# hahnyuan/PTQ4ViT

Measured on AMD Instinct MI355X. Metric: calibration throughput (wrapped modules calibrated per second), ViT-B/224 W8A8, 32 calibration images, higher is better.
Workload: dtype int8

## Files before the change

include/ptq4vit_hip_debug.h:

```cpp
#ifndef PTQ4VIT_HIP_DEBUG_H
#define PTQ4VIT_HIP_DEBUG_H

#include <stdint.h>

#ifdef __cplusplus
extern "C" {
#endif

int p4v_debug_set_variant(int variant, int force_generic);
int p4v_debug_set_tuning(int key, int value);
int p4v_debug_topk_rows(const float* d_mass, int segs, int n, int k, int32_t* d_idx, void* stream);

#ifdef __cplusplus
}
#endif
#endif
```

ptq4vit_amd/_lib.py:

```python
import ctypes as C
import os

_HERE = os.path.dirname(os.path.abspath(__file__))
LIB_PATH = os.environ.get("P4V_LIB") or os.path.join(_HERE, "csrc", "libptq4vit_hip.so")

METRICS = {
    "L1_norm": 0,
    "L2_norm": 1,
    "linear_weighted_L2_norm": 2,
    "square_weighted_L2_norm": 3,
    "hessian": 4,
    "cosine": 5,
}


class LinearDesc(C.Structure):
    _fields_ = [(n, C.c_int32) for n in (
        "batch", "tokens", "in_features", "out_features", "n_V", "n_H", "n_a", "w_bit", "a_bit", "metric",
        "eq_n", "search_round", "twin_postgelu", "init_layerwise", "has_bias", "reserved")]


class MatMulDesc(C.Structure):
    _fields_ = ([(n, C.c_int32) for n in ("batch", "heads", "M", "K", "N")] + [("_pad0", C.c_int32)] +
                [("a_stride", C.c_int64 * 4), ("b_stride", C.c_int64 * 4)] +
# ... 16 lines not shown
                ("memo_hits", C.c_int64), ("memo_misses", C.c_int64),
                ("sweep7_ms", C.c_double), ("sweep7_launches", C.c_int64), ("sweep7_macs", C.c_double), ("sweep7_alg_macs", C.c_double),
                ("sweep7_twin_ms", C.c_double), ("sweep7_twin_launches", C.c_int64), ("event_overhead_ms", C.c_double)]


class LaunchRecord(C.Structure):
    _fields_ = [("kind", C.c_int32), ("stage", C.c_int32), ("grid_x", C.c_int32), ("grid_z", C.c_int32),
                ("ms", C.c_double), ("ops", C.c_double), ("alg_ops", C.c_double), ("alg_bytes", C.c_double)]


LAUNCH_KINDS = {0: "k_sweep<int8>", 1: "k_sweep<float>", 2: "k_sweep6", 3: "k_sweep7", 4: "k_sweep7 (twin)", 5: "k_sweep4/5", 6: "k_sweep9",
                7: "k_sweep8", 8: "k_sweep2g", 9: "k_sweep2", 11: "k_sos_split", 12: "k_bound", 13: "k_slice_b", 14: "k_slice_a"}
LAUNCH_STAGES = {0: "full", 1: "A", 2: "B1", 3: "B2", 4: "A2"}


class PlaneDesc(C.Structure):
    _fields_ = [("rows", C.c_int64), ("cols", C.c_int64), ("cols_padded", C.c_int64), ("rows_per_scale", C.c_int64),
                ("mode", C.c_int32), ("lo", C.c_int32), ("hi", C.c_int32), ("qmax", C.c_int32),
                ("const_scale", C.c_float), ("reserved", C.c_int32)]


class ExportDesc(C.Structure):
    _fields_ = [("dims", C.c_int32 * 4), ("src_stride", C.c_int64 * 4),
                ("scale1_stride", C.c_int64 * 4), ("scale1_div", C.c_int32 * 4),
                ("scale2_stride", C.c_int64 * 4), ("scale2_div", C.c_int32 * 4),
                ("scale2_const", C.c_float),
                ("mode", C.c_int32), ("lo1", C.c_int32), ("hi1", C.c_int32), ("lo2", C.c_int32), ("hi2", C.c_int32),
                ("qmax", C.c_int32), ("reserved", C.c_int32)]


class GroupJob(C.Structure):
    _fields_ = [("kind", C.c_int32), ("status", C.c_int32), ("desc", C.c_void_p), ("inp", C.c_void_p * 5), ("mult", C.c_void_p),
                ("out", C.c_void_p * 3), ("workspace", C.c_void_p), ("workspace_bytes", C.c_size_t)]


JOB_LINEAR, JOB_MATMUL, JOB_CONV = 0, 1, 2
PLANE_SYM, PLANE_SOS_HI, PLANE_SOS_LO, PLANE_TWIN = 1, 2, 3, 4
EXPORT_SYM_I8, EXPORT_SYM_F32, EXPORT_GELU_U8, EXPORT_SOS_U8 = 0, 1, 2, 3


EXPORTS = [
    "p4v_version", "p4v_last_error",
    "p4v_linear_workspace_bytes", "p4v_linear_calibrate",
    "p4v_matmul_workspace_bytes", "p4v_matmul_calibrate",
    "p4v_conv_workspace_bytes", "p4v_conv_calibrate",
    "p4v_calibrate_group", "p4v_launch_counters",
    "p4v_linear_quant_forward", "p4v_matmul_quant_forward",
    "p4v_amax_init_linear", "p4v_linear_search_w", "p4v_linear_search_a",
    "p4v_amax_init_matmul", "p4v_matmul_search_A", "p4v_sos_search_split", "p4v_matmul_search_B",
    "p4v_amax_init_conv", "p4v_conv_search_w_channelwise", "p4v_conv_search_w_layerwise", "p4v_conv_search_a",
    "p4v_score_argmax_gather",
    "p4v_quantize_i8", "p4v_pack_plane_i8", "p4v_fake_quant", "p4v_export_quantize", "p4v_multi_copy",
    "p4v_stats_enable", "p4v_stats_reset", "p4v_stats_get", "p4v_stats_launches", "p4v_prune_counters",
    "p4v_debug_set_variant", "p4v_debug_set_tuning", "p4v_debug_topk_rows",
]

_lib = None


def load():
    global _lib
    if _lib is not None:
        return _lib
    if not os.path.exists(LIB_PATH):
        raise RuntimeError(
            f"ptq4vit_amd: HIP extension {LIB_PATH} is missing -- build it with "
            "`python -c 'import __graft_entry__ as g; g.build()'` (hipcc --offload-arch=gfx950). "
            "There is no CPU fallback for the calibration path.")
    import torch
    lib = C.CDLL(LIB_PATH)
    vp, fp, ip = C.c_void_p, C.c_void_p, C.c_void_p
    lib.p4v_version.restype = C.c_int
    lib.p4v_last_error.restype = C.c_char_p
    lib.p4v_linear_workspace_bytes.restype = C.c_size_t
    lib.p4v_linear_workspace_bytes.argtypes = [C.POINTER(LinearDesc)]
    lib.p4v_linear_calibrate.restype = C.c_int
    lib.p4v_linear_calibrate.argtypes = [C.POINTER(LinearDesc), fp, fp, fp, fp, fp, fp, fp, fp, fp, ip, vp, C.c_size_t, vp]
    lib.p4v_matmul_workspace_bytes.restype = C.c_size_t
    lib.p4v_matmul_workspace_bytes.argtypes = [C.POINTER(MatMulDesc)]
    lib.p4v_matmul_calibrate.restype = C.c_int
    lib.p4v_matmul_calibrate.argtypes = [C.POINTER(MatMulDesc), fp, fp, fp, fp, fp, fp, fp, fp, fp, ip, vp, C.c_size_t, vp]
    lib.p4v_conv_workspace_bytes.restype = C.c_size_t
    lib.p4v_conv_workspace_bytes.argtypes = [C.POINTER(ConvDesc)]
    lib.p4v_conv_calibrate.restype = C.c_int
    lib.p4v_conv_calibrate.argtypes = [C.POINTER(ConvDesc), fp, fp, fp, fp, fp, fp, fp, fp, fp, ip, vp, C.c_size_t, vp]
    lib.p4v_linear_quant_forward.restype = C.c_int
    lib.p4v_linear_quant_forward.argtypes = [C.POINTER(LinearDesc), fp, fp, fp, fp, fp, fp, vp, C.c_size_t, vp]
    lib.p4v_matmul_quant_forward.restype = C.c_int
    lib.p4v_matmul_quant_forward.argtypes = [C.POINTER(MatMulDesc), fp, fp, fp, fp, fp, fp, vp, C.c_size_t, vp]
    LD, MD, CD = C.POINTER(LinearDesc), C.POINTER(MatMulDesc), C.POINTER(ConvDesc)
    tail = [vp, C.c_size_t, vp]
    for name, args in (
            ("p4v_amax_init_linear", [LD] + [fp] * 4),
            ("p4v_linear_search_w", [LD] + [fp] * 9 + [ip]),
            ("p4v_linear_search_a", [LD] + [fp] * 9 + [ip]),
            ("p4v_amax_init_matmul", [MD] + [fp] * 4),
            ("p4v_matmul_search_A", [MD] + [fp] * 8 + [ip]),
            ("p4v_sos_search_split", [MD] + [fp] * 7 + [ip]),
            ("p4v_matmul_search_B", [MD] + [fp] * 9 + [ip]),
            ("p4v_amax_init_conv", [CD] + [fp] * 4),
            ("p4v_conv_search_w_channelwise", [CD] + [fp] * 9 + [ip]),
            ("p4v_conv_search_w_layerwise", [CD] + [fp] * 9 + [ip]),
            ("p4v_conv_search_a", [CD] + [fp] * 9 + [ip])):
        fn = getattr(lib, name)
        fn.restype = C.c_int
        fn.argtypes = args + tail
    lib.p4v_score_argmax_gather.restype = C.c_int
    lib.p4v_score_argmax_gather.argtypes = [fp, C.c_int32, C.c_int32, fp, fp, ip, vp]
    lib.p4v_quantize_i8.restype = C.c_int
    lib.p4v_quantize_i8.argtypes = [fp, C.c_int64, C.c_int64, C.c_int64, fp, C.c_int64, C.c_int32, C.c_int32, vp, vp]
    lib.p4v_fake_quant.restype = C.c_int
    lib.p4v_fake_quant.argtypes = [fp, C.c_int64, C.c_int64, fp, C.c_int64, C.c_int32, C.c_int32, fp, vp]
    lib.p4v_pack_plane_i8.restype = C.c_int
    lib.p4v_pack_plane_i8.argtypes = [C.POINTER(PlaneDesc), fp, fp, vp, vp]
    lib.p4v_export_quantize.restype = C.c_int
    lib.p4v_export_quantize.argtypes = [C.POINTER(ExportDesc), fp, fp, fp, vp, vp]
    lib.p4v_multi_copy.restype = C.c_int
    lib.p4v_multi_copy.argtypes = [vp, C.c_int32, C.c_int64, C.c_int64, vp]
    lib.p4v_debug_topk_rows.restype = C.c_int
    lib.p4v_debug_topk_rows.argtypes = [vp, C.c_int, C.c_int, C.c_int, vp, vp]
    lib.p4v_debug_set_variant.restype = C.c_int
    lib.p4v_debug_set_variant.argtypes = [C.c_int, C.c_int]
    lib.p4v_debug_set_tuning.restype = C.c_int
    lib.p4v_debug_set_tuning.argtypes = [C.c_int, C.c_int]
    lib.p4v_stats_enable.restype = C.c_int
    lib.p4v_stats_enable.argtypes = [C.c_int]
    lib.p4v_stats_reset.restype = C.c_int
    lib.p4v_stats_get.restype = C.c_int
    lib.p4v_stats_get.argtypes = [C.POINTER(KernelStats)]
    lib.p4v_stats_launches.restype = C.c_int
    lib.p4v_stats_launches.argtypes = [C.POINTER(LaunchRecord), C.c_int64, C.POINTER(C.c_int64)]
    lib.p4v_prune_counters.restype = C.c_int
    lib.p4v_prune_counters.argtypes = [C.POINTER(C.c_int64), C.c_int]
    lib.p4v_launch_counters.restype = C.c_int
    lib.p4v_launch_counters.argtypes = [C.POINTER(C.c_int64), C.c_int]
    lib.p4v_calibrate_group.restype = C.c_int
    lib.p4v_calibrate_group.argtypes = [C.POINTER(GroupJob), C.c_int32, vp, vp]
    _lib = lib
    return lib


def check(rc, what):
    if rc != 0:
        msg = load().p4v_last_error().decode("utf-8", "replace")
        if rc == -2:
            raise NotImplementedError(f"{what}: {msg}")
        raise RuntimeError(f"{what} failed (code {rc}): {msg}")


def source_hash():
    import hashlib
    root = os.path.dirname(os.path.abspath(__file__))
    h = hashlib.sha256()
    for rel in ("csrc/p4v_kernels.h", "csrc/p4v_api.hip", "../include/ptq4vit_hip.h"):
        with open(os.path.join(root, rel), "rb") as f:
            h.update(f.read())
    return h.hexdigest()[:16]
```

ptq4vit_amd/csrc/p4v_api.hip:

```cpp
#include <hip/hip_runtime.h>

#include <algorithm>
#include <atomic>
#include <climits>
#include <cstdarg>
#include <cstdio>
#include <condition_variable>
#include <cstring>
#include <deque>
#include <functional>
#include <thread>
#include <mutex>
#include <string>
#include <unordered_map>
#include <type_traits>
#include <vector>

#include "../../include/ptq4vit_hip.h"
#include "../../include/ptq4vit_hip_debug.h"
#include "p4v_kernels.h"

using namespace p4v;

namespace {
// ... 906 lines not shown
    const int cos6_slabs = ps.cos7 ? Np / 128 : ps.cos6 ? (a_search ? Np / 64 : (int)cdiv(ps.Ncols, 64)) : 0;
    const long p_zs = (ps.cos6 || ps.cos7) ? (long)cos6_slabs * cos6_Sp * 3 : stat_ok ? (long)s3_slabs * s3_groups : big7 ? (long)MT7 * NpP : (long)MT * NpP * (cosm ? 3 : 1);
    const long p_cs = p_zs * ps.Z;
    float* part = c.ws.get<float>((size_t)p_cs * ps.eq_n);
    float* S1 = !ps.use_s1 ? nullptr : ps.S1_pre ? ps.S1_pre : c.ws.get<float>((size_t)ps.eq_n * ps.s_cs);
    float* S2 = !(ps.use_s1 && ps.twin) ? nullptr : ps.S2_pre ? ps.S2_pre : c.ws.get<float>((size_t)ps.eq_n * ps.s_cs);
    float* scores = ps.scores_keep ? ps.scores_keep : c.ws.get<float>((size_t)ps.eq_n * std::max(1, ps.nj));
    float* zero_bias = (stat_ok && !ps.bias) ? c.ws.get<float>((size_t)std::max(Mp, Np)) : nullptr;
    float* epi7 = big7 ? c.ws.get<float>((size_t)Mp * Np * 2) : nullptr;
    const int s6_stiles = (a_search ? Np : Mp) / 256, s6_ttiles = (int)cdiv(a_search ? ps.Mrows : ps.Ncols, 64);
    const bool epi6_on = regs6 && (a_search || ps.cos6 || tune(TUNE_EPI6W) == 1);
    const size_t epi6_bytes = epi6_on ? (size_t)s6_stiles * s6_ttiles * (256 * 64 * 8) : 0;
    EpiCache* ec = (epi6_on && ps.ecache && (long)epi6_bytes <= PLANE_CACHE_MAX) ? ps.ecache : nullptr;
    if (ec && !ec->assigned) {
        ec->buf = c.ws.get_top(epi6_bytes);
        ec->assigned = true; ec->valid = false;
    }
    float* epi6 = !epi6_on ? nullptr : ec ? reinterpret_cast<float*>(ec->buf) : c.ws.get<float>(epi6_bytes / 4);
    if (!c.ws.ok()) return fail(P4V_ERR_WORKSPACE, "workspace too small: need >= %zu bytes", c.ws.off);
    auto pack = [&](Operand& op, char* buf, int Rp, bool shared, int c0, int nc) -> int {
        PackParams pk = op.pk;
        pk.Rp = Rp; pk.Kp = Kp; pk.dst = buf;
        pk.Z = shared ? 1 : ps.Z;
        pk.C = op.expanded ? nc : 1;
        pk.c_inner = (stat_ok && op.expanded) ? (pairs ? 2 : 1) : 0;
        if (regs6 && !op.expanded) pk.c_inner = 3;
        if (bound) pk.c_inner = 3;
        if (op.expanded && pk.scales) pk.scales += (long)c0 * pk.sc_cs;
        if (op.expanded && ps.crange) {
            pk.crange = ps.crange; pk.c_base = c0;
            pk.done = (pc && pc->done) ? pc->done : nullptr;
        }
        CHK(ps.i8 ? launch_pack<int8_t>(c, pk) : launch_pack<float>(c, pk));
        return 0;
    };
    if (ps.pack_only) {
        if (pc && !pc->valid && ps.row.expanded != ps.col.expanded && !ps.crange) {
            if (ps.row.expanded) CHK(pack(ps.row, rowbuf, Mp, ps.row_zs_shared, 0, ps.eq_n));
            else CHK(pack(ps.col, colbuf, NpB, ps.col_zs_shared, 0, ps.eq_n));
            pc->valid = true;
            if (!c.dry && pc->done) CHK(q_fill(c, pc->done, 1, (size_t)ps.eq_n));
        }
        c.ws.off = mark;
        return 0;
    }
    if (epi6_on && !c.dry && !(ec && ec->valid)) {
        PrepEpi6Params pe{};
        pe.O = ps.O; pe.Wt = ps.G ? ps.G : ps.O; pe.bias = ps.bias ? ps.bias : zero_bias;
        pe.o_ss = a_search ? ps.o_ns : ps.o_ms; pe.o_ts = a_search ? ps.o_ms : ps.o_ns;
        pe.SR = a_search ? ps.Ncols : ps.Mrows; pe.TR = a_search ? ps.Mrows : ps.Ncols;
        pe.bias_on_t = a_search ? 0 : 1; pe.wt_mode = ps.cos6 ? 4 : ps.wt_mode;
        pe.stiles = s6_stiles; pe.ttiles = s6_ttiles; pe.E = epi6; pe.transposed = (ps.cos6 && !a_search) ? 1 : 0;
        if (zero_bias) CHK(q_fill(c, zero_bias, 0, sizeof(float) * (size_t)std::max(Mp, Np)));
        const long chunks = (long)(epi6_bytes / 16);
        CHK(enqueue(c, KERN(PrepEpi6Params, k_prep_epi6), dim3((unsigned)std::min<long>(cdiv(chunks, 256), 256L * 32)), dim3(256), 0, pe));
    }
    if (ec) ec->valid = true;
    if (big7 && !c.dry) {
        PrepEpiParams pe{ps.O, ps.G ? ps.G : ps.O, ps.bias, ps.o_ms, ps.Mrows, ps.Ncols, ps.cos7 ? 4 : ps.wt_mode,
                         Np / 256, Mp / (ps.twin ? 128 : 256), ps.twin ? 1 : 0, epi7};
        const long chunks = (long)Mp * Np * 2 / 4;
        CHK(enqueue(c, KERN(PrepEpiParams, k_prep_epi), dim3((unsigned)std::min<long>(cdiv(chunks, 256), 256L * 16)), dim3(256), 0, pe));
    }

    if (zero_bias && !c.dry) CHK(q_fill(c, zero_bias, 0, sizeof(float) * (size_t)std::max(Mp, Np)));
    if (ps.use_s1 && !ps.s_ready) {
        ps.s1.S = S1; ps.s1.C = ps.eq_n; ps.s1.nblk = ps.s_cs;
        CHK(launch_scale(c, ps.s1));
        if (ps.twin) { ps.s2.S = S2; ps.s2.C = ps.eq_n; ps.s2.nblk = ps.s_cs; CHK(launch_scale(c, ps.s2)); }
    }
    if (merged7) {
        Operand both = ps.row;
        both.pk.mode = PACK_TWIN_I8;
        both.pk.lo = ps.row2.pk.lo; both.pk.neg_scale = ps.row2.pk.neg_scale;
        CHK(pack(both, rowbuf, Mp, ps.row_zs_shared, 0, 1));
    } else if (ps.twin && ps.i8 && !ps.row.expanded && !ps.row2.expanded && dual_pack_ok(ps.row.pk, ps.row2.pk)) {
        PackParams p1 = ps.row.pk, p2 = ps.row2.pk;
        p1.Rp = p2.Rp = Mp; p1.Kp = p2.Kp = Kp; p1.Z = p2.Z = ps.row_zs_shared ? 1 : ps.Z; p1.C = p2.C = 1;
        p1.dst = rowbuf; p2.dst = row2buf;
        if (!c.dry) {
            const long total = (long)p1.Z * Mp * (Kp / 16);
            if (total >= (1L << 31)) return fail(P4V_ERR_UNSUPPORTED, "operand plane too large for k_pack_dual (%ld 16-element runs)", total);
            CHK(enqueue(c, KERN(PackDualParams, k_pack_dual), dim3((unsigned)std::min<long>(cdiv(total, 256), 256L * 64)), dim3(256), 0, PackDualParams{p1, p2}));
        }
    } else {
        if (!ps.row.expanded) CHK(pack(ps.row, rowbuf, Mp, ps.row_zs_shared, 0, 1));
        if (ps.twin && !ps.row2.expanded) CHK(pack(ps.row2, row2buf, Mp, ps.row_zs_shared, 0, 1));
    }
    if (!ps.col.expanded) CHK(pack(ps.col, colbuf, NpB, ps.col_zs_shared, 0, 1));

    int nine_halves = 0;
    for (int c0 = 0; c0 < ps.eq_n; c0 += chunk) {
        const int nc = std::min(chunk, ps.eq_n - c0);
        const bool packed = pc && pc->valid;
        if (ps.row.expanded && !packed) CHK(pack(ps.row, rowbuf, Mp, ps.row_zs_shared, c0, nc));
        if (ps.twin && ps.row2.expanded) CHK(pack(ps.row2, row2buf, Mp, ps.row_zs_shared, c0, nc));
        if (ps.col.expanded && !packed) CHK(pack(ps.col, colbuf, NpB, ps.col_zs_shared, c0, nc));
        if (pc && !ps.crange && !packed) {
            pc->valid = true;
            if (!c.dry && pc->done) CHK(q_fill(c, pc->done, 1, (size_t)ps.eq_n));
        }
        if (g_stat_on && ps.crange && !c.dry) {
            int h[2] = {0, 0};
            const bool host_knows = ps.host_hi > ps.host_lo;
            const bool one_cand = !host_knows && g_stage == 2 && ps.nj == 1;
            if (host_knows) { h[0] = ps.host_lo; h[1] = ps.host_hi; }
            else if (one_cand) { h[0] = c0; h[1] = c0 + 1; }
            else { CHK(q_d2h(c, h, ps.crange, sizeof h)); CHK(q_sync(c)); }
// ... 1820 lines not shown
    g_stat_done.clear();
    g_memo_hits = 0; g_memo_misses = 0;
    return r;
}

int p4v_stats_get(p4v_kernel_stats* out) {
    if (!out) return fail(P4V_ERR_INVALID, "stats_get: null");
    int r = stats_drain();
    g_stats.memo_hits = g_memo_hits; g_stats.memo_misses = g_memo_misses;
    g_stats.event_overhead_ms = g_evt_overhead_ms;
    *out = g_stats;
    return r;
}

int p4v_stats_launches(p4v_launch_record* out, int64_t capacity, int64_t* count) {
    int r = stats_drain();
    if (r) return r;
    if (count) *count = (int64_t)g_stat_done.size();
    if (out)
        for (int64_t i = 0; i < capacity && i < (int64_t)g_stat_done.size(); ++i) {
            const StatRec& s = g_stat_done[(size_t)i];
            out[i] = p4v_launch_record{s.kind, s.stage, s.gx, s.gz, (double)s.ms, 2.0 * s.macs, 2.0 * s.alg, s.bytes};
        }
    return 0;
}

int p4v_prune_counters(int64_t* out4, int reset) {
    if (out4) for (int i = 0; i < 4; ++i) out4[i] = (int64_t)g_prune_cnt[i].load(std::memory_order_relaxed);
    if (reset) for (int i = 0; i < 4; ++i) g_prune_cnt[i].store(0, std::memory_order_relaxed);
    return 0;
}

int p4v_debug_set_variant(int variant, int force_generic) {
    if (variant < 0 || variant >= (1 << 30)) return fail(P4V_ERR_INVALID, "p4v_debug_set_variant: bad variant word");
    if (variant & ~VARIANT_KEPT) return fail(P4V_ERR_INVALID, "p4v_debug_set_variant: bits 0x%x select removed paths", variant & ~VARIANT_KEPT);
    g_variant_word.store(variant | (force_generic ? (1 << 30) : 0), std::memory_order_relaxed);
    return 0;
}

int p4v_debug_set_tuning(int key, int value) {
    if (key < 0 || key >= 16) return fail(P4V_ERR_INVALID, "p4v_debug_set_tuning: unknown key %d", key);
    if (key == TUNE_B1_PATH && tune_b1_removed(value)) return fail(P4V_ERR_INVALID, "p4v_debug_set_tuning: 12 = %d selects a removed path", value);
    g_tune[key].store(value, std::memory_order_relaxed);
    return 0;
}

int p4v_debug_topk_rows(const float* d_mass, int segs, int n, int k, int32_t* d_idx, void* stream) {
    if (!d_mass || !d_idx || segs <= 0 || n <= 0 || k <= 0 || k > n) return fail(P4V_ERR_INVALID, "p4v_debug_topk_rows: bad argument");
    hipLaunchKernelGGL(k_topk_rows, dim3(segs), dim3(1024), 0, (hipStream_t)stream, TopkParams{d_mass, n, k, d_idx});
    HIPCHK(hipGetLastError());
    return 0;
}

int p4v_pack_plane_i8(const p4v_plane_desc* d, const float* d_x, const float* d_scales, int8_t* d_q, void* stream) {
    if (!d || !d_x || !d_q || d->rows <= 0 || d->cols <= 0 || d->cols_padded % 64 || d->cols_padded < d->cols)
        return fail(P4V_ERR_INVALID, "p4v_pack_plane_i8: bad argument");
    if (d->mode != P4V_PLANE_SYM && d->mode != P4V_PLANE_SOS_HI && d->mode != P4V_PLANE_SOS_LO && d->mode != P4V_PLANE_TWIN)
        return fail(P4V_ERR_INVALID, "p4v_pack_plane_i8: unknown mode %d", d->mode);
    if (d->mode == P4V_PLANE_TWIN && (d->lo > 0 || d->hi < 0 || !(d->const_scale > 0.0f)))
        return fail(P4V_ERR_INVALID, "p4v_pack_plane_i8: the merged twin plane needs lo <= 0 <= hi and const_scale > 0");
    if (d->mode != P4V_PLANE_SYM && !d_scales) return fail(P4V_ERR_INVALID, "p4v_pack_plane_i8: split-of-softmax planes need d_scales = &split");
    if (d->mode == P4V_PLANE_SYM && d_scales && d->rows_per_scale <= 0) return fail(P4V_ERR_INVALID, "p4v_pack_plane_i8: rows_per_scale");
    if (d->lo < -128 || d->hi > 127 || d->qmax < 2 || d->qmax > 128) return fail(P4V_ERR_INVALID, "p4v_pack_plane_i8: grid wider than int8");
    Ctx c{(hipStream_t)stream, Arena(nullptr, 0), false};
    cvt_bias(c);
    PackParams p = pack2d(d_x, d->rows, d->cols, d->cols);
    p.Rp = (int)d->rows; p.Kp = (int)d->cols_padded; p.dst = d_q; p.C = 1;
    p.scales = d_scales; p.sc_cs = 0; p.neg_scale = d->const_scale;
    p.lo = d->lo; p.hi = d->hi; p.qm1 = (float)(d->qmax - 1);
    if (d->mode == P4V_PLANE_SYM) {
        p.mode = PACK_SYM;
        if (d_scales) { p.blk_mode = 1; p.blk_div = (int)d->rows_per_scale; p.nblk_r = cdiv(d->rows, d->rows_per_scale); p.nblk_k = 1; }
    } else if (d->mode == P4V_PLANE_TWIN) {
        p.mode = PACK_TWIN_I8;
    } else {
        p.mode = d->mode == P4V_PLANE_SOS_HI ? PACK_SOS_HI : PACK_SOS_LO;
    }
    return launch_pack<int8_t>(c, p);
}

int p4v_export_quantize(const p4v_export_desc* d, const float* d_src, const float* d_scale1, const float* d_scale2,
                        void* d_dst, void* stream) {
    if (!d || !d_src || !d_scale1 || !d_dst) return fail(P4V_ERR_INVALID, "p4v_export_quantize: null pointer");
    if (d->mode < P4V_EXPORT_SYM_I8 || d->mode > P4V_EXPORT_SOS_U8) return fail(P4V_ERR_INVALID, "p4v_export_quantize: unknown mode %d", d->mode);
    if (d->mode == P4V_EXPORT_SOS_U8 && !d_scale2) return fail(P4V_ERR_INVALID, "p4v_export_quantize: the split-of-softmax format needs d_scale2 = A_interval");
    ExportParams p{};
    long total = 1;
    for (int i = 0; i < 4; ++i) {
        if (d->dims[i] <= 0 || d->scale1_div[i] <= 0 || (d_scale2 && d->scale2_div[i] <= 0))
            return fail(P4V_ERR_INVALID, "p4v_export_quantize: non-positive dimension / block size");
        p.d[i] = d->dims[i]; p.ss[i] = d->src_stride[i];
        p.s1s[i] = d->scale1_stride[i]; p.s1d[i] = d->scale1_div[i];
        p.s2s[i] = d->scale2_stride[i]; p.s2d[i] = d_scale2 ? d->scale2_div[i] : 1;
        total *= d->dims[i];
    }
    p.src = d_src; p.s1 = d_scale1; p.s2 = d_scale2; p.s2_const = d->scale2_const;
    p.mode = d->mode == P4V_EXPORT_SYM_I8 ? EXP_SYM_I8 : d->mode == P4V_EXPORT_SYM_F32 ? EXP_SYM_F32
           : d->mode == P4V_EXPORT_GELU_U8 ? EXP_GELU_U8 : EXP_SOS_U8;
    p.lo1 = d->lo1; p.hi1 = d->hi1; p.lo2 = d->lo2; p.hi2 = d->hi2; p.qm1 = (float)(d->qmax - 1);
    p.dst = d_dst;
    const unsigned blocks = (unsigned)std::min<long>(cdiv(total, 256), 256L * 32);
    hipLaunchKernelGGL(k_export, dim3(blocks), dim3(256), 0, (hipStream_t)stream, p);
    HIPCHK(hipGetLastError());
    return 0;
}

// ... 2 lines not shown
```

ptq4vit_amd/csrc/p4v_kernels.h:

```cpp
#pragma once
#include <hip/hip_runtime.h>
#include <stdint.h>
#include <type_traits>

namespace p4v {

typedef int v4i __attribute__((ext_vector_type(4)));
typedef int v16i __attribute__((ext_vector_type(16)));
typedef float v4f __attribute__((ext_vector_type(4)));
typedef float v16f __attribute__((ext_vector_type(16)));
typedef float v2f __attribute__((ext_vector_type(2)));

#ifndef P4V_GROUP_KERNARG
#define P4V_GROUP_KERNARG (4096 - 256)
#endif
template <typename P> struct GroupArgs {
    static constexpr int CAP_RAW = (P4V_GROUP_KERNARG - 16) / (int)(sizeof(P) + 16);
    static constexpr int CAP = CAP_RAW > 64 ? 64 : CAP_RAW;
    int n;
    unsigned off[CAP + 1];
    unsigned gx[CAP], gy[CAP], gz[CAP];
    P p[CAP];
};
#define P4V_BIDX uint3{blockIdx.x, blockIdx.y, blockIdx.z}
// ... 345 lines not shown
                    for (int e = 0; e < 16; ++e) qb[e] = quant_fast1(x[e], rcp, flo - 0.49f, fhi + 0.49f, magic, maxdev);
                    const bool bad = !(maxdev <= 0.49996f) || !(rcp < 3.0e38f) || !(fmaxf(-flo, fhi) < 129.0f);
                    if (__any(bad)) {
                        float sd = s;
                        asm volatile("" : "+v"(sd));
                        if (bad) {
#pragma unroll
                            for (int e = 0; e < 16; ++e)
                                qb[e] = __builtin_bit_cast(unsigned, fminf(fmaxf(rintf(x[e] / sd), flo), fhi) + PACK_MAGIC);
                        }
                    }
#pragma unroll
                    for (int q = 0; q < 4; ++q) {
                        const unsigned lo16 = __builtin_amdgcn_perm(qb[q * 4 + 1], qb[q * 4], 0x0c0c0400u);
                        const unsigned hi16 = __builtin_amdgcn_perm(qb[q * 4 + 3], qb[q * 4 + 2], 0x0c0c0400u);
                        w[q] = (int)(lo16 | (hi16 << 16));
                    }
                } else {
#pragma unroll
                    for (int q = 0; q < 4; ++q) {
                        int acc = 0;
#pragma unroll
                        for (int e = 0; e < 4; ++e) {
                            const int kk = kc * 16 + q * 4 + e;
                            float v = (live && kk < p.K) ? pack_value(p, x[q * 4 + e], s) : 0.0f;
                            acc |= ((int)v & 0xff) << (8 * e);
                        }
                        w[q] = acc;
                    }
                }
                __builtin_nontemporal_store(v4i{w[0], w[1], w[2], w[3]}, reinterpret_cast<v4i*>(reinterpret_cast<int8_t*>(p.dst) + o));
            } else {
                float* d = reinterpret_cast<float*>(p.dst) + o;
#pragma unroll
                for (int q = 0; q < 4; ++q) {
                    v4f v;
#pragma unroll
                    for (int e = 0; e < 4; ++e) {
                        const int kk = kc * 16 + q * 4 + e;
                        const float s = !p.scales ? 1.0f : per_k_blk ? p.scales[c * p.sc_cs + blk[q * 4 + e]] : sc[j];
                        v[e] = (live && kk < p.K) ? pack_value_f32(p, x[q * 4 + e], s) : 0.0f;
                    }
                    *reinterpret_cast<v4f*>(d + q * 4) = v;
                }
            }
        }
    }
}
template <typename T>
__global__ __launch_bounds__(256) void k_pack(PackParams p) { k_pack_body<T>(p, P4V_BIDX, P4V_GDIM); }
template <typename T>
__global__ __launch_bounds__(256) void k_pack_g(GroupArgs<PackParams> a) { P4V_GROUP_ENTER(a); k_pack_body<T>(a.p[m_], vb_, vg_); }

__device__ __forceinline__ void k_pack_twin_body(const PackParams& p, const uint3 blockIdx, const uint3 gridDim) {
    const unsigned kchunks = p.Kp / 16;
    const unsigned total = (unsigned)p.Z * p.Rp * kchunks;
    const float s = p.scales[0], sn = p.neg_scale, flo = (float)p.lo, fhi = (float)p.hi;
    for (unsigned i = blockIdx.x * 256u + threadIdx.x; i < total; i += gridDim.x * 256u) {
        const unsigned row = i / kchunks;
        const int kc = (int)(i - row * kchunks);
        const int z = (int)(row / (unsigned)p.Rp);
        const int r = (int)(row - (unsigned)z * p.Rp);
        const float* zbase = p.src + (long)z * p.s_z;
        int w[4];
#pragma unroll
        for (int q = 0; q < 4; ++q) {
            int acc = 0;
#pragma unroll
            for (int e = 0; e < 4; ++e) {
                const int k = kc * 16 + q * 4 + e;
                const float x = pack_load(p, zbase, r, k);
                const float v = fminf(fmaxf(rintf(x / s), 0.0f), fhi) + fminf(fmaxf(rintf(x / sn), flo), 0.0f);
                acc |= ((int)v & 0xff) << (8 * e);
            }
            w[q] = acc;
        }
        *reinterpret_cast<v4i*>(reinterpret_cast<int8_t*>(p.dst) + (((long)z * p.Rp + r) * p.Kp + (long)kc * 16)) = v4i{w[0], w[1], w[2], w[3]};
    }
}
__global__ __launch_bounds__(256) void k_pack_twin(PackParams p) { k_pack_twin_body(p, P4V_BIDX, P4V_GDIM); }
__global__ __launch_bounds__(256) void k_pack_twin_g(GroupArgs<PackParams> a) { P4V_GROUP_ENTER(a); k_pack_twin_body(a.p[m_], vb_, vg_); }


struct PackDualParams { PackParams p; PackParams p2; };
__device__ __forceinline__ void k_pack_dual_body(const PackDualParams& a_, const uint3 blockIdx, const uint3 gridDim) {
    const auto& [p, p2] = a_;
    const unsigned kchunks = p.Kp / 16;
    const unsigned total = (unsigned)p.Z * p.Rp * kchunks;
    const float s1 = p.scales ? p.scales[0] : p.neg_scale, s2 = p2.scales ? p2.scales[0] : p2.neg_scale;
    for (unsigned i = blockIdx.x * 256u + threadIdx.x; i < total; i += gridDim.x * 256u) {
        const unsigned row = i / kchunks;
        const int kc = (int)(i - row * kchunks);
        const int z = (int)(row / (unsigned)p.Rp);
        const int r = (int)(row - (unsigned)z * p.Rp);
        const float* zbase = p.zdiv > 0 ? p.src + (long)(z / p.zdiv) * p.s_z2 + (long)(z % p.zdiv) * p.s_z
                                        : p.src + (long)z * p.s_z;
        float x[16];
        const bool vec = p.s_k == 1 && r < p.R && kc * 16 + 16 <= p.K && (p.s_r & 3) == 0 && ((((unsigned long long)zbase) & 15) == 0);
        if (vec) {
            const v4f* src4 = reinterpret_cast<const v4f*>(zbase + (long)r * p.s_r + kc * 16);
#pragma unroll
            for (int q = 0; q < 4; ++q) {
                const v4f t = src4[q];
                x[q * 4 + 0] = t[0]; x[q * 4 + 1] = t[1]; x[q * 4 + 2] = t[2]; x[q * 4 + 3] = t[3];
            }
        } else {
#pragma unroll
            for (int e = 0; e < 16; ++e) x[e] = pack_load(p, zbase, r, kc * 16 + e);
        }
        const bool live = r < p.R;
        int w1[4], w2[4];
#pragma unroll
        for (int q = 0; q < 4; ++q) {
            int a1 = 0, a2 = 0;
#pragma unroll
            for (int e = 0; e < 4; ++e) {
                const bool in = live && kc * 16 + q * 4 + e < p.K;
                const float v1 = in ? pack_value(p, x[q * 4 + e], s1) : 0.0f;
                const float v2 = in ? pack_value(p2, x[q * 4 + e], s2) : 0.0f;
                a1 |= ((int)v1 & 0xff) << (8 * e);
                a2 |= ((int)v2 & 0xff) << (8 * e);
            }
            w1[q] = a1; w2[q] = a2;
        }
        const long o = ((long)z * p.Rp + r) * p.Kp + (long)kc * 16;
        __builtin_nontemporal_store(v4i{w1[0], w1[1], w1[2], w1[3]}, reinterpret_cast<v4i*>(reinterpret_cast<int8_t*>(p.dst) + o));
        __builtin_nontemporal_store(v4i{w2[0], w2[1], w2[2], w2[3]}, reinterpret_cast<v4i*>(reinterpret_cast<int8_t*>(p2.dst) + o));
    }
}
__global__ __launch_bounds__(256) void k_pack_dual(PackDualParams p) { k_pack_dual_body(p, P4V_BIDX, P4V_GDIM); }
__global__ __launch_bounds__(256) void k_pack_dual_g(GroupArgs<PackDualParams> a) { P4V_GROUP_ENTER(a); k_pack_dual_body(a.p[m_], vb_, vg_); }

__global__ void k_fake_quant_rows(const float* x, long rows, long cols, const float* scales, long rows_per_scale,
                                  float lo, float hi, float* y) {
    const long n = rows * cols;
    for (long i = (long)blockIdx.x * blockDim.x + threadIdx.x; i < n; i += (long)gridDim.x * blockDim.x) {
        const float s = scales[(i / cols) / rows_per_scale];
        y[i] = fminf(fmaxf(rintf(x[i] / s), lo), hi) * s;
    }
}

__global__ __launch_bounds__(256) void k_multi_copy(const long* table, long index) {
    const long* e = table + 3 * (long)blockIdx.y;
    const char* src = reinterpret_cast<const char*>(e[0]);
    const long bytes = e[2];
    char* dst = reinterpret_cast<char*>(e[1]) + index * bytes;
    if (((e[0] | (long)(size_t)dst | bytes) & 15) == 0) {
        const long n = bytes >> 4;
        for (long i = (long)blockIdx.x * 256 + threadIdx.x; i < n; i += (long)gridDim.x * 256)
            reinterpret_cast<v4i*>(dst)[i] = reinterpret_cast<const v4i*>(src)[i];
    } else {
        const long n = bytes >> 2;
        for (long i = (long)blockIdx.x * 256 + threadIdx.x; i < n; i += (long)gridDim.x * 256)
            reinterpret_cast<int*>(dst)[i] = reinterpret_cast<const int*>(src)[i];
    }
}

enum ExportMode {
    EXP_SYM_I8 = 0,
    EXP_SYM_F32 = 1,
    EXP_GELU_U8 = 2,
    EXP_SOS_U8 = 3
// ... 1639 lines not shown
            kt = 0;
            cidx += 2;
        }
    };
    auto step = [&](Frag& cur, Frag& nxt) __attribute__((always_inline)) {
        wait_vmcnt<2>();
        __builtin_amdgcn_s_barrier();
        glds16(curT, smem + issue_base + is_stage);
        glds16(curT + SW_BKB, smem + issue_base + is_stage + SW2_TILE);
        curT += 2 * SW_BKB;
        is_stage = (is_stage + PST == SW5_NP * PST) ? 0 : is_stage + PST;
        read_frags(nxt);
        mma(cur);
        __builtin_amdgcn_s_waitcnt(0xC07F);
    };
#ifdef P4V_TRACE
    if (threadIdx.x == 0) trc[1] = __builtin_amdgcn_s_memrealtime();
#endif
    wait_vmcnt<4>();
    __builtin_amdgcn_s_barrier();
#ifdef P4V_TRACE
    if (threadIdx.x == 0) trc[6] = __builtin_amdgcn_s_memrealtime();
#endif
    read_frags(fa);
    __builtin_amdgcn_s_waitcnt(0xC07F);
    int it = 0;
    for (; it + 1 < total; it += 2) { step(fa, fb); step(fb, fa); }
    if (it < total) step(fa, fb);
#ifdef P4V_TRACE
    if (threadIdx.x == 0) trc[2] = __builtin_amdgcn_s_memrealtime();
#endif
    __syncthreads();
    for (int i = tid; i < (c_hi - c_lo) * 8; i += 512) {
        const int cc = c_lo + i / 8, wv = i % 8;
        p.part[(long)cc * p.p_cs + (long)(st * 2 + (wv >> 2)) * p.NG + tt * 4 + (wv & 3)] = res[i];
    }
#ifdef P4V_TRACE
    if (threadIdx.x == 0) { trc[3] = __builtin_amdgcn_s_memrealtime(); trc[7] = (unsigned long long)total; trc[9] = __builtin_amdgcn_s_memtime(); }
#endif
}
template <int EPI>
__global__ __launch_bounds__(512, 2) void k_sweep5(Sweep3Params p) { k_sweep5_body<EPI>(p, P4V_BIDX, P4V_GDIM); }
template <int EPI>
__global__ __launch_bounds__(512, 2) void k_sweep5_g(GroupArgs<Sweep3Params> a) { P4V_GROUP_ENTER(a); k_sweep5_body<EPI>(a.p[m_], vb_, vg_); }

struct PrepEpi6Params {
    const float* O; const float* Wt; const float* bias;
    long o_ss, o_ts; int SR, TR, bias_on_t, wt_mode;
    int stiles, ttiles;
    float* E;
    int transposed;
};
__device__ __forceinline__ void k_prep_epi6_body(const PrepEpi6Params& p, const uint3 blockIdx, const uint3 gridDim) {
    const long total = (long)p.stiles * p.ttiles * 8 * 2 * 4 * 2 * 64;
    for (long i = (long)blockIdx.x * 256 + threadIdx.x; i < total; i += (long)gridDim.x * 256) {
        const int lane = (int)(i & 63), k = (int)((i >> 6) & 1), q = (int)((i >> 7) & 3), cb = (int)((i >> 9) & 1), b = (int)((i >> 10) & 7);
        const long t = i >> 13;
        const int st = (int)(t % p.stiles), tt = (int)(t / p.stiles);
        const int g = lane >> 5, l31 = lane & 31;
        const int tr0 = tt * 64 + cb * 32 + (p.transposed ? 8 * q + 4 * g : l31);
        const int sr0 = st * 256 + b * 32 + (p.transposed ? l31 : 8 * q + 4 * g);
        v4f v = {0.f, 0.f, 0.f, 0.f};
#pragma unroll
        for (int e = 0; e < 4; ++e) {
            const int sr = sr0 + (p.transposed ? 0 : e), tr = tr0 + (p.transposed ? e : 0);
            if (sr < p.SR && tr < p.TR) {
                const long idx = (long)sr * p.o_ss + (long)tr * p.o_ts;
                const float o = p.O[idx];
                const float bs = p.bias[p.bias_on_t ? tr : sr];
                if (k == 0) v[e] = p.wt_mode == 4 ? o : o - bs;
                else v[e] = p.wt_mode == 1 ? p.Wt[idx] : p.wt_mode == 2 ? o : p.wt_mode == 3 ? fabsf(o) : p.wt_mode == 4 ? bs : 1.0f;
            }
        }
        reinterpret_cast<v4f*>(p.E)[i] = v;
    }
}
__global__ __launch_bounds__(256) void k_prep_epi6(PrepEpi6Params p) { k_prep_epi6_body(p, P4V_BIDX, P4V_GDIM); }
__global__ __launch_bounds__(256) void k_prep_epi6_g(GroupArgs<PrepEpi6Params> a) { P4V_GROUP_ENTER(a); k_prep_epi6_body(a.p[m_], vb_, vg_); }

#ifndef P4V_SW6_DBG
#define P4V_SW6_DBG 0
#endif
template <int EPI, int KT, int RB>
__device__ __forceinline__ void k_sweep6_body(const Sweep3Params& p, const uint3 blockIdx, const uint3 gridDim) {
    constexpr int NW = 8 / RB;
    constexpr bool COS = EPI == EPI_COS || EPI == EPI_COS_T, TR = EPI == EPI_COS_T;
    static_assert(RB == 2, "k_sweep6: one wave per SIMD (RB = 2) only");
    extern __shared__ __attribute__((aligned(16))) char smem[];
#ifdef P4V_TRACE
    unsigned long long* trc = p.trace + ((size_t)blockIdx.z * gridDim.x + blockIdx.x) * 16;
    if (threadIdx.x == 0) { trc[0] = __builtin_amdgcn_s_memrealtime(); trc[8] = __builtin_amdgcn_s_memtime(); trc[5] = __builtin_amdgcn_s_getreg((20 << 0) | (0 << 6) | (31 << 11)); }
#endif
    constexpr int KT_TILE = 64 * 64;
    constexpr int STG = KT * KT_TILE;
    float* res = reinterpret_cast<float*>(smem + 3 * STG);

    const int tid = threadIdx.x, lane = tid & 63;
    const int wid = __builtin_amdgcn_readfirstlane(tid >> 6);
    const int g = lane >> 5, l31 = lane & 31;

    const int nwg = p.ntile > 0 ? p.ntile : p.stiles * p.ttiles;
    const int t = p.tile0 + xcd_remap(blockIdx.x, nwg);
    const int st = t % p.stiles, tt = t / p.stiles;
    const int s0 = st * 256 + wid * (32 * RB), t0 = tt * 64;
    const int per = (p.c1 - p.c0 + gridDim.z - 1) / gridDim.z;
    int c_lo_ = p.c0 + blockIdx.z * per, c_hi_ = min(p.c1, c_lo_ + per);
    clip_crange(p.crange, c_lo_, c_hi_);
    if (p.crange_blk) clip_crange_blk(p.crange_blk, min((p.sb_on_t ? tt * 64 : st * 256) / p.sb_div, p.s_cs - 1), c_lo_, c_hi_);
    const int c_lo = c_lo_, c_hi = c_hi_;
    if (c_lo >= c_hi) return;
    const int ncand = c_hi - c_lo;

    constexpr int NPC = 4 * KT;
    constexpr int PPW = (NPC + NW - 1) / NW;
    const int ld_row = (wid & 3) * 16 + (lane >> 2);
    const int ld_chunk = (lane & 3) ^ ((ld_row >> 2) & 3);
    const char* curT = (const char*)p.T + (long)(t0 + ld_row) * p.t_rs + (long)(c_lo - p.c0) * p.ldk + ld_chunk * 16;
    const int kt_w = wid >> 2;
    curT += kt_w * SW_BKB;
    auto piece = [&](const char* src, int stage_off, auto j_c) __attribute__((always_inline)) {
        constexpr int j = decltype(j_c)::value;
        constexpr int OFF = j * (NW / 4) * SW_BKB;
        const int kt = j * (NW / 4) + kt_w;
        if (NPC % NW == 0 || NW * j + wid < NPC)
            glds16_imm<OFF>(src, smem + stage_off + kt * KT_TILE + (wid & 3) * 1024 - OFF);
    };
    auto issue = [&](int stage_off) __attribute__((always_inline)) {
// ... 1374 lines not shown
```

ptq4vit_amd/engine.py:

```python
import ctypes as C

import torch

from . import _lib

_workspace = {}
_mult_cache = {}


def _require_cuda(t, what):
    if not t.is_cuda:
        raise RuntimeError(f"ptq4vit_amd: {what} must live on the GPU (got {t.device}); the calibration path has no CPU fallback")


def device_of(*tensors):
    for t in tensors:
        if t is not None and t.is_cuda:
            return t.device
    if not torch.cuda.is_available():
        raise RuntimeError("ptq4vit_amd: no GPU visible -- the HIP calibration engine needs an MI355X (no CPU fallback)")
    return torch.device("cuda", torch.cuda.current_device())


def to_dev(t, dev):
# ... 495 lines not shown
    if src.dtype != torch.float32:
        if src_stride is not None and not src.is_contiguous():
            raise TypeError("export_quantize: explicit src_stride needs a float32 source (convert before deriving the strides)")
        src = src.float()
    if dims is None:
        dims, src_stride = _pad4(src.shape, 1), _pad4(src.stride(), 0)
    code = {"sym_i8": _lib.EXPORT_SYM_I8, "sym_f32": _lib.EXPORT_SYM_F32, "gelu_u8": _lib.EXPORT_GELU_U8,
            "sos_u8": _lib.EXPORT_SOS_U8}[mode]
    out = torch.empty(tuple(dims), dtype={"sym_i8": torch.int8, "sym_f32": torch.float32}.get(mode, torch.uint8), device=dev)
    d = _lib.ExportDesc()
    for i in range(4):
        d.dims[i], d.src_stride[i] = int(dims[i]), int(src_stride[i])
        d.scale1_stride[i], d.scale1_div[i] = int(scale1_stride[i]), int(scale1_div[i])
        d.scale2_stride[i], d.scale2_div[i] = int(scale2_stride[i]), int(scale2_div[i])
    d.scale2_const = float(scale2_const)
    d.mode, d.lo1, d.hi1, d.lo2, d.hi2, d.qmax, d.reserved = code, int(lo1), int(hi1), int(lo2), int(hi2), int(qmax), 0
    s1 = to_dev(torch.as_tensor(scale1), dev).reshape(-1).contiguous()
    s2 = to_dev(torch.as_tensor(scale2), dev).reshape(-1).contiguous() if scale2 is not None else None
    with torch.cuda.device(dev):
        rc = lib.p4v_export_quantize(C.byref(d), ptr(src), ptr(s1), ptr(s2), ptr(out), stream_ptr(dev))
    _lib.check(rc, "p4v_export_quantize")
    return out


def multi_copy(table, n, index, max_bytes, dev):
    lib = _lib.load()
    with torch.cuda.device(dev):
        rc = lib.p4v_multi_copy(ptr(table), int(n), int(index), int(max_bytes), stream_ptr(dev))
    _lib.check(rc, "p4v_multi_copy")


def stats_enable(flag):
    _lib.load().p4v_stats_enable(int(bool(flag)))


def debug_variant(variant=0, force_generic=False):
    _lib.check(_lib.load().p4v_debug_set_variant(int(variant), int(bool(force_generic))), "p4v_debug_set_variant")


def debug_tuning(key, value):
    _lib.check(_lib.load().p4v_debug_set_tuning(int(key), int(value)), "p4v_debug_set_tuning")


def debug_topk_rows(mass, k):
    assert mass.is_cuda and mass.dtype == torch.float32 and mass.dim() == 2 and mass.is_contiguous()
    segs, n = mass.shape
    out = torch.empty(segs, int(k), dtype=torch.int32, device=mass.device)
    with torch.cuda.device(mass.device):
        rc = _lib.load().p4v_debug_topk_rows(ptr(mass), segs, n, int(k), ptr(out), stream_ptr(mass.device))
    _lib.check(rc, "p4v_debug_topk_rows")
    return out


def stats_reset():
    _lib.load().p4v_stats_reset()


def stats_get():
    s = _lib.KernelStats()
    _lib.check(_lib.load().p4v_stats_get(C.byref(s)), "p4v_stats_get")
    return {k: getattr(s, k) for k, _ in _lib.KernelStats._fields_}


def prune_counters(reset=False):
    out = (C.c_int64 * 4)()
    _lib.check(_lib.load().p4v_prune_counters(out, int(bool(reset))), "p4v_prune_counters")
    return dict(zip(("staged", "staged_no_survivors", "kept_full_sweep", "not_eligible"), (int(v) for v in out)))


def stats_launches():
    lib = _lib.load()
    n = C.c_int64(0)
    _lib.check(lib.p4v_stats_launches(None, 0, C.byref(n)), "p4v_stats_launches")
    buf = (_lib.LaunchRecord * max(1, n.value))()
    _lib.check(lib.p4v_stats_launches(buf, n.value, C.byref(n)), "p4v_stats_launches")
    return [{"kernel": _lib.LAUNCH_KINDS.get(r.kind, str(r.kind)), "stage": _lib.LAUNCH_STAGES.get(r.stage, str(r.stage)),
             "grid_x": r.grid_x, "grid_z": r.grid_z, "ms": r.ms, "ops": r.ops, "alg_ops": r.alg_ops, "alg_bytes": r.alg_bytes}
            for r in buf[:n.value]]
```

Measured before the change: 634.4.

## Vectorize twin pack and restructure prep_epi6 into per-tile coalesced loads

Rewrites k_prep_epi6 so each block handles one output tile and loads O, Wt and bias as aligned float4 vectors when the layout allows, in place of per-element strided gathers indexed from a flat element index. The launch grid now covers tiles instead of element chunks. The twin pack kernel shares a vectorized 16-element load helper, uses reciprocal-based quant16 paths, combines the two planes with byte-wise arithmetic, and writes with nontemporal stores. Debug entry points for testing dual pack and prep_epi6 are also added. The aim is less memory-access overhead in these preprocessing kernels, at the cost of more code paths and possible rounding differences from multiplying by the reciprocal.

Result: faster. 651.3 (median of 6 runs) (+2.7%).

```diff
diff --git a/include/ptq4vit_hip_debug.h b/include/ptq4vit_hip_debug.h
--- a/include/ptq4vit_hip_debug.h
+++ b/include/ptq4vit_hip_debug.h
@@ -10,6 +10,10 @@
 int p4v_debug_set_variant(int variant, int force_generic);
 int p4v_debug_set_tuning(int key, int value);
 int p4v_debug_topk_rows(const float* d_mass, int segs, int n, int k, int32_t* d_idx, void* stream);
+int p4v_debug_pack_dual(const float* d_x, long rows, long cols, long cols_padded, int sos, int lo, int hi, int qmax,
+                        const float* d_scale, float const_scale, int8_t* d_q1, int8_t* d_q2, void* stream);
+int p4v_debug_prep_epi6(const float* d_o, const float* d_wt, const float* d_bias, long o_ss, long o_ts, int sr, int tr,
+                        int bias_on_t, int wt_mode, int transposed, float* d_e, void* stream);
 
 #ifdef __cplusplus
 }
diff --git a/ptq4vit_amd/_lib.py b/ptq4vit_amd/_lib.py
--- a/ptq4vit_amd/_lib.py
+++ b/ptq4vit_amd/_lib.py
@@ -92,7 +92,7 @@
     "p4v_score_argmax_gather",
     "p4v_quantize_i8", "p4v_pack_plane_i8", "p4v_fake_quant", "p4v_export_quantize", "p4v_multi_copy",
     "p4v_stats_enable", "p4v_stats_reset", "p4v_stats_get", "p4v_stats_launches", "p4v_prune_counters",
-    "p4v_debug_set_variant", "p4v_debug_set_tuning", "p4v_debug_topk_rows",
+    "p4v_debug_set_variant", "p4v_debug_set_tuning", "p4v_debug_topk_rows", "p4v_debug_pack_dual", "p4v_debug_prep_epi6",
 ]
 
 _lib = None
@@ -159,6 +159,10 @@
     lib.p4v_multi_copy.argtypes = [vp, C.c_int32, C.c_int64, C.c_int64, vp]
     lib.p4v_debug_topk_rows.restype = C.c_int
     lib.p4v_debug_topk_rows.argtypes = [vp, C.c_int, C.c_int, C.c_int, vp, vp]
+    lib.p4v_debug_pack_dual.restype = C.c_int
+    lib.p4v_debug_pack_dual.argtypes = [fp, C.c_long, C.c_long, C.c_long, C.c_int, C.c_int, C.c_int, C.c_int, fp, C.c_float, vp, vp, vp]
+    lib.p4v_debug_prep_epi6.restype = C.c_int
+    lib.p4v_debug_prep_epi6.argtypes = [fp, fp, fp, C.c_long, C.c_long, C.c_int, C.c_int, C.c_int, C.c_int, C.c_int, fp, vp]
     lib.p4v_debug_set_variant.restype = C.c_int
     lib.p4v_debug_set_variant.argtypes = [C.c_int, C.c_int]
     lib.p4v_debug_set_tuning.restype = C.c_int
diff --git a/ptq4vit_amd/csrc/p4v_api.hip b/ptq4vit_amd/csrc/p4v_api.hip
--- a/ptq4vit_amd/csrc/p4v_api.hip
+++ b/ptq4vit_amd/csrc/p4v_api.hip
@@ -982,8 +982,7 @@
         pe.bias_on_t = a_search ? 0 : 1; pe.wt_mode = ps.cos6 ? 4 : ps.wt_mode;
         pe.stiles = s6_stiles; pe.ttiles = s6_ttiles; pe.E = epi6; pe.transposed = (ps.cos6 && !a_search) ? 1 : 0;
         if (zero_bias) CHK(q_fill(c, zero_bias, 0, sizeof(float) * (size_t)std::max(Mp, Np)));
-        const long chunks = (long)(epi6_bytes / 16);
-        CHK(enqueue(c, KERN(PrepEpi6Params, k_prep_epi6), dim3((unsigned)std::min<long>(cdiv(chunks, 256), 256L * 32)), dim3(256), 0, pe));
+        CHK(enqueue(c, KERN(PrepEpi6Params, k_prep_epi6), dim3((unsigned)std::min<long>((long)s6_stiles * s6_ttiles, 256L * 32)), dim3(256), 0, pe));
     }
     if (ec) ec->valid = true;
     if (big7 && !c.dry) {
@@ -2910,6 +2909,40 @@
     return 0;
 }
 
+int p4v_debug_pack_dual(const float* d_x, long rows, long cols, long cols_padded, int sos, int lo, int hi, int qmax,
+                        const float* d_scale, float const_scale, int8_t* d_q1, int8_t* d_q2, void* stream) {
+    if (!d_x || !d_scale || !d_q1 || !d_q2 || rows <= 0 || cols <= 0 || cols_padded % 64 || cols_padded < cols ||
+        lo > 0 || hi < 0 || lo < -128 || hi > 127 || qmax < 2 || qmax > 128 || (!sos && !(const_scale > 0.0f)))
+        return fail(P4V_ERR_INVALID, "p4v_debug_pack_dual: bad argument");
+    PackParams p1 = pack2d(d_x, rows, cols, cols);
+    p1.Rp = (int)rows; p1.Kp = (int)cols_padded; p1.C = 1; p1.scales = d_scale; p1.qm1 = (float)(qmax - 1);
+    PackParams p2 = p1;
+    p1.dst = d_q1; p2.dst = d_q2;
+    if (sos) {
+        p1.mode = PACK_SOS_HI; p2.mode = PACK_SOS_LO;
+    } else {
+        p1.lo = 0; p1.hi = hi; p2.lo = lo; p2.hi = 0; p2.scales = nullptr; p2.neg_scale = const_scale;
+    }
+    if (!dual_pack_ok(p1, p2)) return fail(P4V_ERR_INVALID, "p4v_debug_pack_dual: not a dual pair");
+    Ctx c{(hipStream_t)stream, Arena(nullptr, 0), false};
+    const long total = rows * (cols_padded / 16);
+    if (total >= (1L << 31)) return fail(P4V_ERR_UNSUPPORTED, "p4v_debug_pack_dual: plane too large");
+    return enqueue(c, KERN(PackDualParams, k_pack_dual), dim3((unsigned)std::min<long>(cdiv(total, 256), 256L * 64)), dim3(256), 0,
+                   PackDualParams{p1, p2});
+}
+
+int p4v_debug_prep_epi6(const float* d_o, const float* d_wt, const float* d_bias, long o_ss, long o_ts, int sr, int tr,
+                        int bias_on_t, int wt_mode, int transposed, float* d_e, void* stream) {
+    if (!d_o || !d_bias || !d_e || (wt_mode == 1 && !d_wt) || sr <= 0 || tr <= 0 || wt_mode < 0 || wt_mode > 4)
+        return fail(P4V_ERR_INVALID, "p4v_debug_prep_epi6: bad argument");
+    PrepEpi6Params pe{};
+    pe.O = d_o; pe.Wt = d_wt ? d_wt : d_o; pe.bias = d_bias; pe.o_ss = o_ss; pe.o_ts = o_ts; pe.SR = sr; pe.TR = tr;
+    pe.bias_on_t = bias_on_t ? 1 : 0; pe.wt_mode = wt_mode; pe.transposed = transposed ? 1 : 0;
+    pe.stiles = cdiv(sr, 256); pe.ttiles = cdiv(tr, 64); pe.E = d_e;
+    Ctx c{(hipStream_t)stream, Arena(nullptr, 0), false};
+    return enqueue(c, KERN(PrepEpi6Params, k_prep_epi6), dim3((unsigned)std::min<long>((long)pe.stiles * pe.ttiles, 256L * 32)), dim3(256), 0, pe);
+}
+
 int p4v_pack_plane_i8(const p4v_plane_desc* d, const float* d_x, const float* d_scales, int8_t* d_q, void* stream) {
     if (!d || !d_x || !d_q || d->rows <= 0 || d->cols <= 0 || d->cols_padded % 64 || d->cols_padded < d->cols)
         return fail(P4V_ERR_INVALID, "p4v_pack_plane_i8: bad argument");
diff --git a/ptq4vit_amd/csrc/p4v_kernels.h b/ptq4vit_amd/csrc/p4v_kernels.h
--- a/ptq4vit_amd/csrc/p4v_kernels.h
+++ b/ptq4vit_amd/csrc/p4v_kernels.h
@@ -421,30 +421,45 @@
 template <typename T>
 __global__ __launch_bounds__(256) void k_pack_g(GroupArgs<PackParams> a) { P4V_GROUP_ENTER(a); k_pack_body<T>(a.p[m_], vb_, vg_); }
 
+__device__ __forceinline__ void pack_load16(const PackParams& p, const float* zbase, int r, int kc, float (&x)[16]) {
+    const bool vec = !p.conv && p.s_k == 1 && r < p.R && kc * 16 + 16 <= p.K && (p.s_r & 3) == 0 &&
+                     ((((unsigned long long)zbase) & 15) == 0);
+    if (vec) {
+        const v4f* src4 = reinterpret_cast<const v4f*>(zbase + (long)r * p.s_r + kc * 16);
+#pragma unroll
+        for (int q = 0; q < 4; ++q) {
+            const v4f t = src4[q];
+            x[q * 4 + 0] = t[0]; x[q * 4 + 1] = t[1]; x[q * 4 + 2] = t[2]; x[q * 4 + 3] = t[3];
+        }
+    } else {
+#pragma unroll
+        for (int e = 0; e < 16; ++e) x[e] = pack_load(p, zbase, r, kc * 16 + e);
+    }
+}
+
 __device__ __forceinline__ void k_pack_twin_body(const PackParams& p, const uint3 blockIdx, const uint3 gridDim) {
     const unsigned kchunks = p.Kp / 16;
     const unsigned total = (unsigned)p.Z * p.Rp * kchunks;
     const float s = p.scales[0], sn = p.neg_scale, flo = (float)p.lo, fhi = (float)p.hi;
+    const float rs = 1.0f / s, rn = 1.0f / sn;
+    const bool wide = !(fmaxf(-flo, fhi) < 129.0f);
     for (unsigned i = blockIdx.x * 256u + threadIdx.x; i < total; i += gridDim.x * 256u) {
         const unsigned row = i / kchunks;
         const int kc = (int)(i - row * kchunks);
         const int z = (int)(row / (unsigned)p.Rp);
         const int r = (int)(row - (unsigned)z * p.Rp);
-        const float* zbase = p.src + (long)z * p.s_z;
-        int w[4];
+        float x[16];
+        pack_load16(p, p.src + (long)z * p.s_z, r, kc, x);
+        v4i a, b;
+        quant16_any(x, s, rs, 0.0f, fhi, wide, a);
+        quant16_any(x, sn, rn, flo, 0.0f, wide, b);
+        v4i w;
 #pragma unroll
         for (int q = 0; q < 4; ++q) {
-            int acc = 0;
-#pragma unroll
-            for (int e = 0; e < 4; ++e) {
-                const int k = kc * 16 + q * 4 + e;
-                const float x = pack_load(p, zbase, r, k);
-                const float v = fminf(fmaxf(rintf(x / s), 0.0f), fhi) + fminf(fmaxf(rintf(x / sn), flo), 0.0f);
-                acc |= ((int)v & 0xff) << (8 * e);
-            }
-            w[q] = acc;
-        }
-        *reinterpret_cast<v4i*>(reinterpret_cast<int8_t*>(p.dst) + (((long)z * p.Rp + r) * p.Kp + (long)kc * 16)) = v4i{w[0], w[1], w[2], w[3]};
+            const unsigned ua = (unsigned)a[q], ub = (unsigned)b[q];
+            w[q] = (int)(((ua & 0x7f7f7f7fu) + (ub & 0x7f7f7f7fu)) ^ ((ua ^ ub) & 0x80808080u));
+        }
+        __builtin_nontemporal_store(w, reinterpret_cast<v4i*>(reinterpret_cast<int8_t*>(p.dst) + (((long)z * p.Rp + r) * p.Kp + (long)kc * 16)));
     }
 }
 __global__ __launch_bounds__(256) void k_pack_twin(PackParams p) { k_pack_twin_body(p, P4V_BIDX, P4V_GDIM); }
@@ -465,18 +480,7 @@
         const float* zbase = p.zdiv > 0 ? p.src + (long)(z / p.zdiv) * p.s_z2 + (long)(z % p.zdiv) * p.s_z
                                         : p.src + (long)z * p.s_z;
         float x[16];
-        const bool vec = p.s_k == 1 && r < p.R && kc * 16 + 16 <= p.K && (p.s_r & 3) == 0 && ((((unsigned long long)zbase) & 15) == 0);
-        if (vec) {
-            const v4f* src4 = reinterpret_cast<const v4f*>(zbase + (long)r * p.s_r + kc * 16);
-#pragma unroll
-            for (int q = 0; q < 4; ++q) {
-                const v4f t = src4[q];
-                x[q * 4 + 0] = t[0]; x[q * 4 + 1] = t[1]; x[q * 4 + 2] = t[2]; x[q * 4 + 3] = t[3];
-            }
-        } else {
-#pragma unroll
-            for (int e = 0; e < 16; ++e) x[e] = pack_load(p, zbase, r, kc * 16 + e);
-        }
+        pack_load16(p, zbase, r, kc, x);
         const bool live = r < p.R;
         int w1[4], w2[4];
 #pragma unroll
@@ -2222,27 +2226,62 @@
     int transposed;
 };
 __device__ __forceinline__ void k_prep_epi6_body(const PrepEpi6Params& p, const uint3 blockIdx, const uint3 gridDim) {
-    const long total = (long)p.stiles * p.ttiles * 8 * 2 * 4 * 2 * 64;
-    for (long i = (long)blockIdx.x * 256 + threadIdx.x; i < total; i += (long)gridDim.x * 256) {
-        const int lane = (int)(i & 63), k = (int)((i >> 6) & 1), q = (int)((i >> 7) & 3), cb = (int)((i >> 9) & 1), b = (int)((i >> 10) & 7);
-        const long t = i >> 13;
-        const int st = (int)(t % p.stiles), tt = (int)(t / p.stiles);
-        const int g = lane >> 5, l31 = lane & 31;
-        const int tr0 = tt * 64 + cb * 32 + (p.transposed ? 8 * q + 4 * g : l31);
-        const int sr0 = st * 256 + b * 32 + (p.transposed ? l31 : 8 * q + 4 * g);
-        v4f v = {0.f, 0.f, 0.f, 0.f};
-#pragma unroll
-        for (int e = 0; e < 4; ++e) {
-            const int sr = sr0 + (p.transposed ? 0 : e), tr = tr0 + (p.transposed ? e : 0);
-            if (sr < p.SR && tr < p.TR) {
-                const long idx = (long)sr * p.o_ss + (long)tr * p.o_ts;
-                const float o = p.O[idx];
-                const float bs = p.bias[p.bias_on_t ? tr : sr];
-                if (k == 0) v[e] = p.wt_mode == 4 ? o : o - bs;
-                else v[e] = p.wt_mode == 1 ? p.Wt[idx] : p.wt_mode == 2 ? o : p.wt_mode == 3 ? fabsf(o) : p.wt_mode == 4 ? bs : 1.0f;
-            }
-        }
-        reinterpret_cast<v4f*>(p.E)[i] = v;
+    const bool tr_cols = p.transposed != 0;
+    const long rs = tr_cols ? p.o_ss : p.o_ts, cs = tr_cols ? p.o_ts : p.o_ss;
+    const int nrow = tr_cols ? p.SR : p.TR, ncol = tr_cols ? p.TR : p.SR;
+    const bool bias_col = (p.bias_on_t != 0) == tr_cols;
+    const bool wt = p.wt_mode == 1;
+    const bool vec = cs == 1 && (rs & 3) == 0 && bias_col &&
+                     ((((unsigned long long)p.O) | (wt ? (unsigned long long)p.Wt : 0ull) | ((unsigned long long)p.bias)) & 15) == 0;
+    const int lane = threadIdx.x & 63, q = threadIdx.x >> 6, g = lane >> 5, l31 = lane & 31;
+    const int ntiles = p.stiles * p.ttiles;
+    for (int t = blockIdx.x; t < ntiles; t += gridDim.x) {
+        const int st = t % p.stiles, tt = t / p.stiles;
+#pragma unroll 1
+        for (int u0 = 0; u0 < 16; u0 += 4) {
+            v4f o[4], w[4], bs[4];
+            int row[4], col0[4];
+#pragma unroll
+            for (int j = 0; j < 4; ++j) {
+                const int b = (u0 + j) >> 1, cb = (u0 + j) & 1;
+                const int sb = st * 256 + b * 32, tb = tt * 64 + cb * 32;
+                row[j] = (tr_cols ? sb : tb) + l31;
+                col0[j] = (tr_cols ? tb : sb) + 8 * q + 4 * g;
+                o[j] = v4f{0.f, 0.f, 0.f, 0.f}; w[j] = o[j]; bs[j] = o[j];
+                if (row[j] >= nrow) continue;
+                if (vec && col0[j] + 4 <= ncol) {
+                    const long idx = (long)row[j] * rs + col0[j];
+                    o[j] = *reinterpret_cast<const v4f*>(p.O + idx);
+                    if (wt) w[j] = *reinterpret_cast<const v4f*>(p.Wt + idx);
+                    bs[j] = *reinterpret_cast<const v4f*>(p.bias + col0[j]);
+                } else {
+#pragma unroll
+                    for (int e = 0; e < 4; ++e) {
+                        const int col = col0[j] + e;
+                        if (col >= ncol) continue;
+                        const long idx = (long)row[j] * rs + (long)col * cs;
+                        o[j][e] = p.O[idx];
+                        if (wt) w[j][e] = p.Wt[idx];
+                        bs[j][e] = p.bias[bias_col ? col : row[j]];
+                    }
+                }
+            }
+#pragma unroll
+            for (int j = 0; j < 4; ++j) {
+                const int b = (u0 + j) >> 1, cb = (u0 + j) & 1;
+                v4f v0 = {0.f, 0.f, 0.f, 0.f}, v1 = v0;
+#pragma unroll
+                for (int e = 0; e < 4; ++e) {
+                    if (row[j] >= nrow || col0[j] + e >= ncol) continue;
+                    const float x = o[j][e], bx = bs[j][e];
+                    v0[e] = p.wt_mode == 4 ? x : x - bx;
+                    v1[e] = wt ? w[j][e] : p.wt_mode == 2 ? x : p.wt_mode == 3 ? fabsf(x) : p.wt_mode == 4 ? bx : 1.0f;
+                }
+                v4f* E = reinterpret_cast<v4f*>(p.E) + ((((long)(t * 8 + b) * 2 + cb) * 4 + q) * 2) * 64 + lane;
+                E[0] = v0;
+                E[64] = v1;
+            }
+        }
     }
 }
 __global__ __launch_bounds__(256) void k_prep_epi6(PrepEpi6Params p) { k_prep_epi6_body(p, P4V_BIDX, P4V_GDIM); }
diff --git a/ptq4vit_amd/engine.py b/ptq4vit_amd/engine.py
--- a/ptq4vit_amd/engine.py
+++ b/ptq4vit_amd/engine.py
@@ -571,6 +571,30 @@
     return out
 
 
+def debug_pack_dual(x2d, *, sos, scale, lo, hi, qmax, const_scale=0.0):
+    x2d = x2d.contiguous().float()
+    rows, cols = x2d.shape
+    colsp = (cols + 63) // 64 * 64
+    q1 = torch.empty(rows, colsp, dtype=torch.int8, device=x2d.device)
+    q2 = torch.empty_like(q1)
+    sc = torch.tensor([float(scale)], dtype=torch.float32, device=x2d.device)
+    with torch.cuda.device(x2d.device):
+        rc = _lib.load().p4v_debug_pack_dual(ptr(x2d), rows, cols, colsp, int(bool(sos)), int(lo), int(hi), int(qmax), ptr(sc),
+                                             float(const_scale), ptr(q1), ptr(q2), stream_ptr(x2d.device))
+    _lib.check(rc, "p4v_debug_pack_dual")
+    return q1[:, :cols], q2[:, :cols], q1, q2
+
+
+def debug_prep_epi6(o, wt, bias, *, o_ss, o_ts, sr, tr, bias_on_t, wt_mode, transposed):
+    n = -(-sr // 256) * -(-tr // 64) * 256 * 64 * 2
+    e = torch.full((n,), float("nan"), dtype=torch.float32, device=o.device)
+    with torch.cuda.device(o.device):
+        rc = _lib.load().p4v_debug_prep_epi6(ptr(o), ptr(wt) if wt is not None else None, ptr(bias), int(o_ss), int(o_ts),
+                                             int(sr), int(tr), int(bias_on_t), int(wt_mode), int(transposed), ptr(e),
+                                             stream_ptr(o.device))
+    _lib.check(rc, "p4v_debug_prep_epi6")
+    return e
+
 def stats_reset():
     _lib.load().p4v_stats_reset()
 
```
